# mitschabaude/msm-zprize

Hardware: AMD Instinct MI355X
Metric: Mpoint-adds/s (ms per MSM in ms_per_step) (higher is better)
Workload: dtype u32 limbs (28-bit lazy Montgomery, i64 accumulate)

## Files before the change

msm_zprize_amd/_native.py:

```python
import ctypes as C
import os

HERE = os.path.dirname(os.path.abspath(__file__))
LIB_PATH = os.environ.get("MSMZ_LIB") or os.path.join(HERE, "libmsmz.so")

MSMZ_N_STAGES = 8
STAGE_NAMES = ["digits", "scan", "scatter", "plan", "accumulate", "reduce", "final", "total"]


class MsmzOpts(C.Structure):
    _fields_ = [("c", C.c_int32), ("glv", C.c_int32), ("safe", C.c_int32), ("buckets", C.c_int32),
                ("timing", C.c_int32), ("reserved", C.c_int32 * 3)]


class MsmzLog(C.Structure):
    _fields_ = [("stage_ms", C.c_float * MSMZ_N_STAGES), ("c", C.c_int32), ("K", C.c_int32), ("rounds", C.c_int32),
                ("glv", C.c_int32), ("n_entries", C.c_uint64), ("n_pairs", C.c_uint64), ("max_bucket", C.c_uint32),
                ("scatter_launches", C.c_uint32), ("scatter_kernel_ms", C.c_float), ("batch_add_ms", C.c_float * 32)]


MSMZ_SRC_DEVICE, MSMZ_SRC_MONTGOMERY, MSMZ_SRC_DEFAULT_STREAM = 1, 2, 4


class MsmzSrc(C.Structure):
# ... 8 lines not shown
class MsmzCheckResult(C.Structure):
    _fields_ = [("off_curve", C.c_uint64), ("off_subgroup", C.c_uint64), ("first_bad", C.c_uint64)]


class MsmzMul(C.Structure):
    _fields_ = [("points_handle", C.c_uint64), ("first_p", C.c_uint64), ("scalars_handle", C.c_uint64),
                ("first_s", C.c_uint64), ("scalar", C.c_char_p), ("addend_handle", C.c_uint64), ("first_q", C.c_uint64)]


class MsmzTestReduceArgs(C.Structure):
    _fields_ = [("mode", C.c_int32), ("c", C.c_int32), ("nsets", C.c_uint32), ("n_in", C.c_uint32),
                ("nc", C.c_uint32), ("tail_n", C.c_uint32), ("quad16_max", C.c_uint32), ("pairsum_x4_max", C.c_uint32),
                ("points_xy", C.c_char_p), ("points_inf", C.c_char_p), ("n_points", C.c_uint64),
                ("slots_xy", C.c_char_p), ("slots_inf", C.c_char_p), ("n_slots", C.c_uint64),
                ("scale", C.c_char_p), ("loc", C.c_void_p), ("cscan", C.c_void_p),
                ("out_xy", C.c_void_p), ("lines_xy", C.c_void_p)]


class MsmzTestPlanArgs(C.Structure):
    _fields_ = [("nb", C.c_uint32), ("chunk", C.c_uint32), ("nb_main", C.c_uint32), ("chunk_top", C.c_uint32),
                ("tail_skip", C.c_int32), ("reserved", C.c_uint32),
                ("off", C.c_void_p), ("refs", C.c_void_p),
                ("desc_cap", C.c_uint64), ("bfin_cap", C.c_uint64), ("chunk_pairs_cap", C.c_uint64),
                ("meta", C.c_void_p), ("desc", C.c_void_p), ("bfin", C.c_void_p), ("chunk_pairs", C.c_void_p)]


class MsmzTestSortArgs(C.Structure):
    _fields_ = [("scalars_le32", C.c_void_p), ("n", C.c_uint64), ("pts_n", C.c_uint64),
                ("nprob", C.c_uint32), ("factor", C.c_uint32), ("copy_stride", C.c_uint32),
                ("c", C.c_int32), ("glv", C.c_int32), ("force_fallback", C.c_int32), ("scalar_bits", C.c_int32),
                ("allow_fold", C.c_int32),
# ... 48 lines not shown
    "msmz_test_field_limbs": (C.c_int, [C.c_void_p, C.c_int, C.c_void_p, C.c_void_p, C.c_uint64, C.c_void_p,
                                        C.c_char_p]),
    "msmz_test_glv": (C.c_int, [C.c_void_p, C.c_char_p, C.c_uint64, C.c_char_p, C.c_char_p, C.c_char_p]),
    "msmz_test_digits": (C.c_int, [C.c_void_p, C.c_char_p, C.c_uint64, C.c_int, C.c_int, C.c_int, C.c_void_p]),
    "msmz_test_sort": (C.c_int, [C.c_void_p, C.c_char_p, C.c_uint64, C.c_int, C.c_int, C.c_int, C.c_void_p, C.c_void_p,
                                 C.c_uint64, C.c_void_p, C.c_uint64]),
    "msmz_test_sort_ex": (C.c_int, [C.c_void_p, C.POINTER(MsmzTestSortArgs)]),
    "msmz_test_point_raw": (C.c_int, [C.c_void_p, C.c_int, C.c_char_p, C.c_char_p, C.c_char_p, C.c_uint64, C.c_int,
                                      C.c_char_p]),
    "msmz_test_point": (C.c_int, [C.c_void_p, C.c_int, C.c_char_p, C.c_char_p, C.c_char_p, C.c_char_p, C.c_uint64,
                                  C.c_char_p]),
    "msmz_test_batch_add": (C.c_int, [C.c_void_p, C.c_int, C.c_int, C.c_char_p, C.c_char_p, C.c_uint64, C.c_char_p,
                                      C.c_char_p, C.c_uint64, C.c_void_p, C.c_uint64, C.c_uint64, C.c_char_p,
                                      C.POINTER(C.c_uint32)]),
    "msmz_test_reduce": (C.c_int, [C.c_void_p, C.POINTER(MsmzTestReduceArgs)]),
    "msmz_test_plan": (C.c_int, [C.c_void_p, C.POINTER(MsmzTestPlanArgs)]),
}

_lib = None


class MsmzError(RuntimeError):
    def __init__(self, status, where):
        self.status = status
        msg = lib().msmz_strerror(status).decode() if _lib is not None else "?"
        super().__init__(f"{where}: msmz status {status} ({msg})")


def lib():
    global _lib
# ... 17 lines not shown
```

msm_zprize_amd/csrc/engine.h:

```cpp
#pragma once
#include <hip/hip_runtime.h>

#include <chrono>
#include <cstdio>
#include <cstdlib>
#include <cstring>
#include <map>
#include <type_traits>
#include <vector>

#include "../../include/msmz.h"
#include "kernels.h"
#include "gen_kernels.h"
#include "import_kernels.h"
#include "check_kernels.h"
#include "mul_kernels.h"
#include "host64.h"
#include "multi.h"
#include "plan.h"

namespace msmz {

#define MSMZ_HIP(x)                                                                        \
  do {                                                                                     \
// ... 118 lines not shown
    load(p, a, ai);
    load(q, b, bi);
    xyzz_add(r, p, q);
    uint32_t w[2 * NW];
    bool inf = xyzz_to_affine_canon<F>(w, r);
    memcpy(out, w, sizeof(w));
    *oi = inf ? 1 : 0;
  }
  return MSMZ_OK;
}

struct ReduceKnobs {
  uint32_t tail_n;
  uint32_t quad16_max;
  uint32_t pairsum_x4_max;
};

template <class Cfg>
class TestHooks;

template <class Cfg>
class Engine : public IEngine {
  friend class TestHooks<Cfg>;
  using F = typename Cfg::F;
  using Fr = typename Cfg::Fr;
  static constexpr int NW = F::NW;
  static constexpr int RW = 2 * NW;
  static constexpr int XW = 4 * NW;
  static constexpr int FE_BYTES = NW * 4;
  static constexpr bool TE = Cfg::TE;
  static constexpr int PW_WORDS = TE ? 4 * NW : PointFmt<F>::STRIDE;

 public:
  Engine(int curve_id, int device) : curve_id_(curve_id), device_(device) {}

  int init() {
    MSMZ_HIP(hipSetDevice(device_));
    MSMZ_HIP(hipStreamCreateWithFlags(&stream_, hipStreamNonBlocking));
    for (hipEvent_t* e : ev_.all()) MSMZ_HIP(hipEventCreate(e));
    MSMZ_HIP(hipEventCreateWithFlags(&import_ev_, hipEventDisableTiming));
    MSMZ_HIP(hipHostMalloc(&h_meta_, sizeof(MsmMeta)));
    int st;
    if ((st = ensure_host_results((size_t)2 * kMaxWindows * XW))) return st;
    if ((st = raise_lds_limit((const void*)k_fine, "k_fine", kFineLds))) return st;
    if ((st = raise_sort_limits<false, 0>()) || (st = raise_sort_limits<false, 16>()) || (st = raise_sort_limits<false, 17>())) return st;
    if constexpr (Fr::HAS_GLV) {
      if ((st = raise_sort_limits<true, 0>()) || (st = raise_sort_limits<true, 16>())) return st;
    }
    return meta_.ensure(sizeof(MsmMeta) + kTraceBytes * 65536);
  }
 private:
  template <bool GLV, int C>
  int raise_sort_limits() {
    int st;
    if ((st = raise_lds_limit((const void*)k_coarse<Fr, GLV, C>, GLV ? "k_coarse<glv>" : "k_coarse", kCoarseLdsMax))) return st;
    return raise_lds_limit((const void*)k_hist<Fr, GLV, C>, GLV ? "k_hist<glv>" : "k_hist", kHistLdsMax);
  }
  static constexpr size_t kFineLds = ((size_t)(1 << FINE_MAX_BITS) + FINE_STAGE) * 4;
  static constexpr size_t kCoarseLdsMax = (size_t)2 * SORT_MAX_BINS * 4;
  static constexpr size_t kHistLdsMax = (size_t)SORT_MAX_BINS * 4;
#ifdef MSMZ_TRACE
  static constexpr size_t kTraceBytes = 128;
#else
// ... 861 lines not shown
  }

  struct HostTe {
    using Pt = TeExt<F>;
    void set_inf(Pt& p) const { te_set_zero(p); }
    void dbl(Pt& r, const Pt& p) const { te_add(r, p, p); }
    void add_pt(Pt& r, const Pt& a, const Pt& b) const { te_add(r, a, b); }
    void load_pt(Pt& p, const uint32_t* w) const {
      fe_unpack<F>(p.X, w);
      fe_unpack<F>(p.Y, w + NW);
      fe_unpack<F>(p.Z, w + 2 * NW);
      fe_unpack<F>(p.T, w + 3 * NW);
    }
  };

  int finish_msm(const Plan& pl, Run& run, bool two_d, uint8_t* out, int* out_inf, msmz_log* log) {
    mark(run, run.ev.red_end);
    const size_t per_problem = (size_t)(two_d ? 2 : 1) * pl.Keff;
    const std::vector<WindowTerm> terms =
        window_terms(pl.c, pl.K, pl.Keff, (int)pl.F, two_d ? planner_.split_2d(pl).b : -1, pl.fold_shift != 0);
    int st = fetch_window_sums(pl, per_problem);
    if (st) return st;
    const auto t_host = std::chrono::steady_clock::now();
    if (h_meta_->error & 1u) return MSMZ_ERR_DEGENERATE;
    for (uint32_t p = 0; p < pl.nprob; p++) {
      const uint32_t* rp = h_res_ + p * per_problem * XW;
      uint32_t w[RW];
      if constexpr (TE) {
        te_to_affine_canon<F>(w, host_horner(HostTe{}, terms, rp, XW));
        out_inf[p] = 0;
      } else {
        Xyzz<F> fin;
        host64_.to_xyzz(fin, host_horner(host64_, terms, rp, XW));
        out_inf[p] = xyzz_to_affine_canon<F>(w, fin) ? 1 : 0;
      }
      memcpy(out + (size_t)p * RW * 4, w, sizeof(w));
    }
    const float host_ms = std::chrono::duration<float, std::milli>(std::chrono::steady_clock::now() - t_host).count();
    fill_log(log, pl, run, host_ms);
    return MSMZ_OK;
  }

  template <class P>
  int reduce_2d(const Plan& pl, const Split2d& sp, const ReduceKnobs& rk, const uint32_t* d_points, bool basic = false,
                bool summed = false) {
    const R2Geom g = r2_geom(pl, sp);
    int rows = 0;
    if (int st = line_sums_2d<P>(g, rk, d_points, basic, summed, &rows)) return st;
    return weighted_sums_2d<P>(g, rk, rows);
  }
  static R2Geom r2_geom(const Plan& pl, const Split2d& sp) {
    R2Geom g;
    g.L = pl.L;
    g.H = sp.H;
    g.D = sp.D;
    g.NC = sp.NC;
    g.chr = sp.D / sp.NC;
    g.chc = sp.H / sp.NC;
    g.nprob = 2u * pl.nprob * (uint32_t)pl.Keff;
    return g;
  }
  template <class P>
  int line_sums_2d(const R2Geom& g, const ReduceKnobs& rk, const uint32_t* d_points, bool basic, bool summed, int* rows) {
    const uint32_t lines = g.nprob * g.H;
// ... 3 lines not shown
    if ((st = red_[2].ensure((size_t)total * XW * 4))) return st;
    if (basic && summed) {
      hipLaunchKernelGGL((k_reduce2d_partial_acc<P>), dim3((total + 127) / 128), dim3(128), 0, stream_,
                         red_[0].as<uint32_t>(), bsum_.as<uint32_t>(), (const uint32_t*)nullptr, g, total);
    } else if (basic) {
      hipLaunchKernelGGL((k_reduce2d_partial_acc<P>), dim3((total + 127) / 128), dim3(128), 0, stream_,
                         red_[0].as<uint32_t>(), slots_.as<uint32_t>(), rscan_.as<uint32_t>(), g, total);
    } else {
      if constexpr (!TE)
        hipLaunchKernelGGL((k_reduce2d_partial<F>), dim3((total + 127) / 128), dim3(128), 0, stream_,
                           red_[0].as<uint32_t>(), slots_.as<uint32_t>(), d_points, bfin_.as<uint4>(), g, total);
    }
    int src = 0;
    for (uint32_t n = total / 2; n >= lines && g.NC > 1; n /= 2) {
      const int dst = src ^ 2;
      if (n <= rk.pairsum_x4_max) {
        hipLaunchKernelGGL((k_pairsum_x4<P>), dim3((n * 4 + 63) / 64), dim3(64), 0, stream_, red_[dst].as<uint32_t>(),
                           red_[src].as<uint32_t>(), n);
      } else {
        hipLaunchKernelGGL((k_pairsum<P>), dim3((n + 127) / 128), dim3(128), 0, stream_, red_[dst].as<uint32_t>(),
                           red_[src].as<uint32_t>(), n);
      }
      src = dst;
      if (n == lines) break;
    }
    *rows = src;
    return MSMZ_OK;
  }
  template <class P>
  int weighted_sums_2d(const R2Geom& g, const ReduceKnobs& rk, int crow) {
    const uint32_t lines = g.nprob * g.H;
    const int ccol = crow + 1;
    int st;
    if ((st = red_[ccol].ensure((size_t)lines * XW * 4))) return st;
    hipLaunchKernelGGL((k_fill_neutral<P>), dim3((lines + 255) / 256), dim3(256), 0, stream_, red_[ccol].as<uint32_t>(), lines);
    int cur = crow >> 1;
    if ((st = reduce_levels<P>(rk, cur, g.H, g.nprob))) return st;
    MSMZ_HIP(hipGetLastError());
    return MSMZ_OK;
  }
  static void fill_log(msmz_log* log, const Plan& pl, const Run& run, float host_ms) {
    if (!log) return;
    log->c = pl.c;
    log->K = pl.K;
    log->rounds = (int)run.rounds;
    log->glv = pl.glv ? 1 : 0;
    log->n_entries = run.n_entries;
    log->n_pairs = run.n_pairs;
// ... 80 lines not shown
      if (pairs == 0) continue;
      launch_batch_add(pairs, opt.safe != 0, d_points, desc_.as<uint2>() + run.round_base[r], run.round_base[r], d_meta);
#ifdef MSMZ_TRACE
      {
        char nm[32];
        snprintf(nm, sizeof nm, "k_batch_add round %d", r);
        const int B = batch_b(pairs);
        const uint32_t wgs = (pairs + MSMZ_BATCH_T * B - 1) / (MSMZ_BATCH_T * B);
        if ((st = trace_dump(nm, d_meta + 1, wgs < 65536 ? wgs : 65536, false))) return st;
      }
#endif
      mark(run, run.ev.round_end[r]);
    }
    mark(run, run.ev.acc_end);

    if (want_2d) {
      if ((st = reduce_2d<WeierPolicy<F>>(pl, planner_.split_2d(pl), reduce_knobs_, d_points))) return st;
    } else {
      uint32_t S1 = planner_.first_group_size(pl);
      if (S1 > 8) S1 = 8;
      while (S1 > 1 && S1 * 2 > pl.L) S1 >>= 1;
      const uint32_t groups = (pl.L + S1 - 1) / S1;
      if ((st = red_[0].ensure((size_t)pl.Keff * groups * XW * 4))) return st;
      if ((st = red_[1].ensure((size_t)pl.Keff * groups * XW * 4))) return st;
      if ((st = reduce_first_affine(pl, d_points, S1, groups, run.n_pairs, d_meta))) return st;
      int cur = 0;
      if ((st = reduce_levels<WeierPolicy<F>>(reduce_knobs_, cur, groups, (uint32_t)pl.Keff))) return st;
    }
    return finish_msm(pl, run, want_2d, out, out_inf, log);
  }

  int msm_basic(const Handle& pts, const uint32_t* d_points, const uint32_t* d_scalars, uint64_t n64, const msmz_opts& opt,
                uint8_t* out, int* out_inf, msmz_log* log) {
    using P = typename std::conditional<TE, TePolicy<F>, WeierPolicy<F>>::type;
    if (opt.glv) return MSMZ_ERR_UNSUPPORTED;
    Plan pl;
    int st = planner_.make_plan(pl, n64, false, opt, (uint32_t)pts.n, false);
    if (st) return st;
    Run run = new_run(opt);
    if ((st = sort_phase(pl, planner_.sort_layout(pl), d_scalars, run, 0)) || (st = fetch_meta(run))) return st;
    if (h_meta_->error & 4u) return MSMZ_ERR_RANGE;
    run.n_pairs = run.n_entries;
    if ((st = partials_.ensure((size_t)32 * pl.nblocks * 4))) return st;
    constexpr int AW = P::ACC_WORDS;
// ... 11 lines not shown
    hipLaunchKernelGGL(k_scan_apply, dim3(nblocks, 1), dim3(SCAN_T), 0, stream_, rscan_.as<uint32_t>(),
                       partials_.as<uint32_t>(), off_.as<uint32_t>(), nb, scan_mode, nblocks, (size_t)0, (uint32_t*)nullptr);
    MSMZ_HIP(hipMemcpyAsync(h_meta_, d_meta, sizeof(MsmMeta), hipMemcpyDeviceToHost, stream_));
    MSMZ_HIP(hipStreamSynchronize(stream_));
    const uint32_t n_chunks = h_meta_->round_pairs[0];
    mark(run, run.ev.plan_end);
    if ((st = slots_.ensure((size_t)(n_chunks + 1) * AW * 4))) return st;
    if (n_chunks > 0) {
      hipLaunchKernelGGL((k_bucket_accumulate<P>), dim3((n_chunks + 127) / 128), dim3(128), 0, stream_,
                         slots_.as<uint32_t>(), d_points, refs_.as<uint32_t>(), off_.as<uint32_t>(),
                         rscan_.as<uint32_t>(), nb, n_chunks, chunk_shift);
    }
    mark(run, run.ev.acc_end);
    const bool summed = (uint64_t)n_chunks * 2 > (uint64_t)nb * 3 && !no_bucket_sums_;
    if (summed && (st = bucket_sums<P>(nb))) return st;
    if ((st = reduce_2d<P>(pl, planner_.split_2d(pl), reduce_knobs_, d_points, true, summed))) return st;
    return finish_msm(pl, run, true, out, out_inf, log);
  }
  template <class P>
  int bucket_sums(uint32_t nb) {
    if (int st = bsum_.ensure((size_t)nb * P::ACC_WORDS * 4)) return st;
    hipLaunchKernelGGL((k_bucket_sums<P>), dim3((nb + 127) / 128), dim3(128), 0, stream_, bsum_.as<uint32_t>(),
                       slots_.as<uint32_t>(), rscan_.as<uint32_t>(), nb);
    return MSMZ_OK;
  }

  int reduce_first_affine(const Plan& pl, const uint32_t* d_points, uint32_t S, uint32_t groups, uint64_t tree_pairs,
                          MsmMeta* d_meta) {
    F2Geom g;
    memset(&g, 0, sizeof(g));
    g.L = pl.L;
    g.S = S;
// ... 136 lines not shown
  int curve_id_, device_;
  hipStream_t stream_ = nullptr;
  StageEvents ev_{};
  hipEvent_t import_ev_ = nullptr;
  std::vector<uint8_t> import_pack_;
  std::map<uint64_t, Handle> handles_;
  uint64_t next_handle_ = 1;
#ifdef MSMZ_DEV
  static int env_int(const char* name, int dflt) { const char* v = getenv(name); return v ? atoi(v) : dflt; }
#else
  static int env_int(const char*, int dflt) { return dflt; }
#endif
  uint32_t batch_min_wgs_ = (uint32_t)env_int("MSMZ_BATCH_WGS", 512);
  int chunk_shift_override_ = env_int("MSMZ_CHUNK_SHIFT", 0);
  const ReduceKnobs reduce_knobs_{(uint32_t)env_int("MSMZ_TAIL_N", REDUCE_TAIL_N), (uint32_t)env_int("MSMZ_QUAD16", 8192),
                                  (uint32_t)env_int("MSMZ_PAIRSUM_X4", 16384)};
  Host64<F> host64_;
  bool no_bucket_sums_ = env_int("MSMZ_NO_BUCKET_SUMS", 0) != 0;
  int tail_skip_2d_ = env_int("MSMZ_TAIL_SKIP_2D", 1) > 2 ? 2 : env_int("MSMZ_TAIL_SKIP_2D", 1);
  int batch_b_override_ = env_int("MSMZ_BATCH_B", 0);
  int retries_ = 0;
  Planner<Fr> planner_{{env_int("MSMZ_NO_SPREAD", 0) != 0, env_int("MSMZ_NO_FOLD", 0) != 0,
                        env_int("MSMZ_NO_WINDOW_MODEL", 0) != 0, env_int("MSMZ_ATOMIC_SORT", 0) != 0,
                        env_int("MSMZ_NO_FBT", 0) != 0, env_int("MSMZ_NO_PLAN_TOP", 0) != 0,
                        env_int("MSMZ_NO_SORT_SPECIAL", 0) != 0, env_int("MSMZ_FB", 0), (uint32_t)env_int("MSMZ_S1", 0),
                        (uint32_t)env_int("MSMZ_R2_NC", 0)}};
  DevBuf bsum_, f2desc_, tilecnt_, tileoff_, final_, desc_, bfin_, packed_, bins_, digits_, counts_, off_, cursor_, refs_, rscan_, partials_, slots_, red_[4], meta_, stage_, gen_table_;
  MsmMeta* h_meta_ = nullptr;
  DevBuf check_;
  CheckResult* h_check_ = nullptr;
  size_t h_check_bytes_ = 0;
  int ensure_host_check(size_t verdict_bytes) {
    const size_t need = sizeof(CheckResult) + verdict_bytes;
    if (need <= h_check_bytes_) return MSMZ_OK;
    if (h_check_) (void)hipHostFree(h_check_);
    h_check_ = nullptr;
    h_check_bytes_ = 0;
    MSMZ_HIP(hipHostMalloc(&h_check_, need));
    h_check_bytes_ = need;
    return MSMZ_OK;
  }
// ... 16 lines not shown
```

msm_zprize_amd/csrc/host64.h:

```cpp
#pragma once
#include <cstdint>
#include <cstring>
#include <vector>

#include "fp.h"

namespace msmz {

template <class F>
struct Fe64 {
  static constexpr int NL = F::NW / 2;
  uint64_t l[NL];
};

template <class F>
struct Host64 {
  static constexpr int NL = F::NW / 2;
  static constexpr int RBITS = F::N * F::W;
  static constexpr int TAIL = RBITS - 64 * NL;
  static_assert(TAIL > 0 && TAIL < 64, "radix must exceed the 64-bit limb length by less than one limb");
  using E = Fe64<F>;
  typedef unsigned __int128 u128;

  uint64_t p[NL];
// ... 218 lines not shown
  }
  std::vector<WindowTerm> t;
  for (int k = K - 1; k >= 0; k--) {
    const int top = k == K - 1 ? Keff - 1 : k;
    if (split_b < 0) {
      for (int kw = top; kw >= k; kw--) t.push_back({c * k, kw});
      continue;
    }
    if (!fold || k < K - 1)
      for (int kw = k; kw <= top; kw++) t.push_back({c * k + split_b, 2 * kw});
    for (int kw = k; kw <= top; kw++) t.push_back({c * k, 2 * kw + 1});
  }
  return t;
}

template <class G>
typename G::Pt host_horner(const G& g, const std::vector<WindowTerm>& terms, const uint32_t* res, int rec_words) {
  typename G::Pt acc, w, t;
  g.set_inf(acc);
  int prev = terms.empty() ? 0 : terms[0].weight;
  for (const WindowTerm& term : terms) {
    for (; prev > term.weight; prev--) {
      g.dbl(t, acc);
      acc = t;
    }
    g.load_pt(w, res + (size_t)term.index * rec_words);
    g.add_pt(t, acc, w);
    acc = t;
  }
  for (; prev > 0; prev--) {
// ... 8 lines not shown
```

msm_zprize_amd/csrc/instantiate.h:

```cpp
#pragma once
#include "check_kernels.h"
#include "gen_kernels.h"
#include "import_kernels.h"
#include "kernels.h"
#include "mul_kernels.h"
#include "test_kernels.h"

#if !defined(MSMZ_CURVE) || MSMZ_CURVE == 0
#define MSMZ_W0(X) X(Bls377Fp, Bls377Fr)
#else
#define MSMZ_W0(X)
#endif
#if !defined(MSMZ_CURVE) || MSMZ_CURVE == 1
#define MSMZ_W1(X) X(PallasFp, PallasFr)
#else
#define MSMZ_W1(X)
#endif
#if !defined(MSMZ_CURVE) || MSMZ_CURVE == 2
#define MSMZ_W2(X) X(Bls381Fp, Bls381Fr)
#else
#define MSMZ_W2(X)
#endif
#if !defined(MSMZ_CURVE) || MSMZ_CURVE == 3
#define MSMZ_T3(X) X(Ed377Fp, Ed377Fr)
// ... 19 lines not shown
  PFX template __global__ void k_batch_add<F, MSMZ_BATCH_T, false, MSMZ_BATCH_OCC, MSMZ_BATCH_BMAX>(             \
      uint32_t*, const uint32_t*, const uint2*, uint32_t, uint32_t, int, MsmMeta*);

#define MSMZ_INST_POLICY(P, PFX)                                                                                 \
  PFX template __global__ void k_reduce_quad<P>(uint32_t*, uint32_t*, const uint32_t*, const uint32_t*, uint32_t, \
                                                uint32_t, uint32_t);                                             \
  PFX template __global__ void k_reduce_quad16<P>(uint32_t*, uint32_t*, const uint32_t*, const uint32_t*,        \
                                                  uint32_t, uint32_t, uint32_t);                                 \
  PFX template __global__ void k_reduce_tail<P>(uint32_t*, uint32_t*, uint32_t*, uint32_t*, uint32_t*, uint32_t, \
                                                uint32_t);                                                       \
  PFX template __global__ void k_pairsum<P>(uint32_t*, const uint32_t*, uint32_t);                               \
  PFX template __global__ void k_fill_neutral<P>(uint32_t*, uint32_t);                                           \
  PFX template __global__ void k_bucket_sums<P>(uint32_t*, const uint32_t*, const uint32_t*, uint32_t);          \
  PFX template __global__ void k_reduce2d_partial_acc<P>(uint32_t*, const uint32_t*, const uint32_t*, R2Geom, uint32_t); \
  PFX template __global__ void k_pairsum_x4<P>(uint32_t*, const uint32_t*, uint32_t);                            \
  PFX template __global__ void k_bucket_accumulate<P>(uint32_t*, const uint32_t*, const uint32_t*,               \
                                                      const uint32_t*, const uint32_t*, uint32_t, uint32_t, int);

#define MSMZ_INST_REDUCE(F, Fr, PFX)                                                                              \
  PFX template __global__ void k_reduce2d_partial<F>(uint32_t*, const uint32_t*, const uint32_t*, const uint4*,   \
                                                     R2Geom, uint32_t);                                          \
  PFX template __global__ void k_reduce_affine_finish<F>(uint32_t*, uint32_t*, const uint32_t*, const uint32_t*,  \
                                                         const uint2*, const uint4*, F2Geom);                     \
  MSMZ_INST_POLICY(WeierPolicy<F>, PFX)

#define MSMZ_INST_REDUCE_TE(F, Fr, PFX) MSMZ_INST_POLICY(TePolicy<F>, PFX)

#define MSMZ_INST_TEST(F, Fr, P, TE, PFX)                                                                         \
  PFX template __global__ void k_test_field<F>(uint32_t*, const uint32_t*, const uint32_t*, uint32_t, int, uint32_t*); \
  PFX template __global__ void k_test_field_limbs<F>(int32_t*, uint32_t*, const int32_t*, const int32_t*, uint32_t,  \
// ... 62 lines not shown
```

msm_zprize_amd/csrc/kernels.h:

```cpp
#pragma once
#include <hip/hip_runtime.h>
#include "constants_gen.h"
#include "plan.h"
#include "curve.h"
#include "scalar.h"

namespace msmz {

constexpr uint32_t REF_NEG = 0x80000000u;
constexpr uint32_t REF_IDX = 0x7fffffffu;

struct MsmMeta {
  uint32_t max_bucket;
  uint32_t n_entries;
  uint32_t error;
  uint32_t rounds;
  uint32_t round_pairs[32];
  uint32_t round_base[32];
};

typedef uint32_t u32x4 __attribute__((ext_vector_type(4)));

#ifndef MSMZ_POINT_PAD
#define MSMZ_POINT_PAD 1
// ... 995 lines not shown
                                                         const uint32_t* c_in, uint32_t n_in, uint32_t groups,
                                                         uint32_t total) {
  constexpr int XW = P::ACC_WORDS;
  const uint32_t t = blockIdx.x * blockDim.x + threadIdx.x;
  const uint32_t grp = t >> 4, q = (t >> 2) & 3;
  const int s = (int)(t & 3);
  const bool live = grp < total;
  const uint32_t k = live ? grp / groups : 0, A = live ? grp - k * groups : 0;
  const int lane = threadIdx.x & 63, base_lane = (lane & ~15) + s;
  reduce_group16<P>(rows_out + (size_t)k * groups * XW, c_out + (size_t)k * groups * XW,
                    rows_in + (size_t)k * n_in * XW, c_in + (size_t)k * n_in * XW, n_in, A, live, q, s, base_lane);
}

constexpr int REDUCE_TAIL_T = 256;
constexpr uint32_t REDUCE_TAIL_N = 32;
template <class P>
__global__ void __launch_bounds__(REDUCE_TAIL_T, 1) k_reduce_tail(uint32_t* r0, uint32_t* c0, uint32_t* r1, uint32_t* c1,
                                                                  uint32_t* c_final, uint32_t n_in, uint32_t stride) {
  constexpr int XW = P::ACC_WORDS;
  const uint32_t k = blockIdx.x;
  uint32_t* rin = r0 + (size_t)k * stride * XW;
  uint32_t* cin = c0 + (size_t)k * stride * XW;
  uint32_t* rout = r1 + (size_t)k * stride * XW;
  uint32_t* cout = c1 + (size_t)k * stride * XW;
  const uint32_t q = (threadIdx.x >> 2) & 3;
  const int s = (int)(threadIdx.x & 3);
  const int lane = threadIdx.x & 63, base_lane = (lane & ~15) + s;
  uint32_t n = n_in;
  while (n > 1) {
    const uint32_t g2 = (n + 3) / 4;
    for (uint32_t A0 = 0; A0 < g2; A0 += REDUCE_TAIL_T / 16) {
      const uint32_t A = A0 + (threadIdx.x >> 4);
      reduce_group16<P>(rout, cout, rin, cin, n, A, A < g2, q, s, base_lane);
    }
    __syncthreads();
    uint32_t* t1 = rin; rin = rout; rout = t1;
    uint32_t* t2 = cin; cin = cout; cout = t2;
    n = g2;
  }
  for (uint32_t j = threadIdx.x; j < (uint32_t)XW; j += REDUCE_TAIL_T) c_final[(size_t)k * XW + j] = cin[j];
}


}

#include "reduce_affine.h"
#include "reduce2d_kernels.h"
```

msm_zprize_amd/csrc/msmz.hip:

```cpp
#include "instantiate.h"
namespace msmz {
#define X(F, Fr) MSMZ_INST_BATCH(F, Fr, MSMZ_EXTERN) MSMZ_INST_REDUCE(F, Fr, MSMZ_EXTERN) MSMZ_INST_MISC(F, Fr, MSMZ_EXTERN) MSMZ_INST_GEN(F, Fr, MSMZ_EXTERN)
MSMZ_WEIERSTRASS_FIELDS(X)
#undef X
#define X(F, Fr) MSMZ_INST_REDUCE_TE(F, Fr, MSMZ_EXTERN) MSMZ_INST_MISC_TE(F, Fr, MSMZ_EXTERN) MSMZ_INST_GEN_TE(F, Fr, MSMZ_EXTERN)
MSMZ_TE_FIELDS(X)
#undef X
}
#include "test_hooks.h"

namespace msmz {

template <class F_, class Fr_>
struct WeierCfg {
  using F = F_;
  using Fr = Fr_;
  static constexpr bool TE = false;
  static constexpr bool HAS_ENDO = true;
};

template <class F_, class Fr_>
struct TeCfg {
  using F = F_;
  using Fr = Fr_;
// ... 207 lines not shown
  return c ? c->engine->test_hooks()->test_point_raw(op, a, b, neg, n, L, out) : MSMZ_ERR_ARG;
}
int msmz_test_point(msmz_ctx* c, int op, const uint8_t* a, const uint8_t* ai, const uint8_t* b, const uint8_t* bi,
                    uint64_t n, uint8_t* out) {
  return c ? c->engine->test_hooks()->test_point(op, a, ai, b, bi, n, out) : MSMZ_ERR_ARG;
}

int msmz_test_batch_add(msmz_ctx* c, int safe, int B, const uint8_t* pxy, const uint8_t* pinf, uint64_t np,
                        const uint8_t* sxy, const uint8_t* sinf, uint64_t ns, const uint32_t* desc, uint64_t n_pairs,
                        uint64_t out_base, uint8_t* out, uint32_t* error) {
  if (!c) return MSMZ_ERR_ARG;
  return c->engine->test_hooks()->test_batch_add(safe, B, pxy, pinf, np, sxy, sinf, ns, desc, n_pairs, out_base, out, error);
}

int msmz_test_reduce(msmz_ctx* c, const msmz_test_reduce_args* a) {
  return c && a ? c->engine->test_hooks()->test_reduce(*a) : MSMZ_ERR_ARG;
}

int msmz_test_plan(msmz_ctx* c, const msmz_test_plan_args* a) {
  return c && a ? c->engine->test_hooks()->test_plan(*a) : MSMZ_ERR_ARG;
}

int msmz_point_add(int curve_id, const uint8_t* a, int ai, const uint8_t* b, int bi, uint8_t* out, int* oi) {
  if (!out || !oi || (!a && !ai) || (!b && !bi)) return MSMZ_ERR_ARG;
  switch (curve_id) {
    case MSMZ_BLS12_377_G1: return host_point_add<Bls377Fp, false>(a, ai, b, bi, out, oi);
    case MSMZ_PALLAS: return host_point_add<PallasFp, false>(a, ai, b, bi, out, oi);
    case MSMZ_BLS12_381_G1: return host_point_add<Bls381Fp, false>(a, ai, b, bi, out, oi);
    case MSMZ_ED_ON_BLS12_377: return host_point_add<Ed377Fp, true>(a, 0, b, 0, out, oi);
    default: return MSMZ_ERR_UNSUPPORTED;
  }
// ... 4 lines not shown
```

msm_zprize_amd/csrc/plan.h:

```cpp
#pragma once
#include <cstdint>
#include <cstring>

#include "../../include/msmz.h"
#include "multi.h"

namespace msmz {

constexpr int COARSE_T = 1024;
constexpr int COARSE_ITEMS = 2;
constexpr int COARSE_TILE = COARSE_T * COARSE_ITEMS;
constexpr int COARSE_MAX_BINS = 512;
constexpr int SORT_MAX_BINS = 8192;
constexpr int FINE_MAX_BITS = 11;
constexpr int FINE_T = 1024;
constexpr int FINE_PER = 37;
constexpr int FINE_STAGE = FINE_T * FINE_PER;

constexpr int PLAN_T = 512;
constexpr int PLAN_PER = 2;
constexpr int PLAN_CHUNK = PLAN_T * PLAN_PER;
constexpr int PLAN_RMAX = 26;

constexpr int SCAN_T = 256;
// ... 60 lines not shown
  uint32_t nprob = 1;
  uint32_t F = 1;
  int sbits = 0;
};

struct Geometry {
  int c, K, t_top, spread, Keff;
  uint32_t L;
  uint32_t top_range = 0;
  int fold_shift = 0, fold_rows = 0;
};

struct Split2d {
  int a, b;
  uint32_t H, D, NC;
};

struct SortLayout {
  SortGeom geom{};
  uint32_t nbins = 0, fbins = 0, fine_top = 0;
  int cspec = 0;
  bool fits = false, two_level = false;
};

struct PlanKnobs {
  bool no_spread = false, no_fold = false, no_window_model = false, force_atomic_sort = false;
  bool no_fbt = false;
  bool no_plan_top = false;
  bool no_sort_special = false;
  int fb_cap = 0;
  uint32_t s1_override = 0, r2_nc = 0;
  int glv_bits_assumed = 0;
};

template <class Fr>
struct Planner {
  PlanKnobs k;

  static int bound(int bits) { return bits <= 0 || bits >= Fr::BITS ? 0 : bits; }

  int scalar_bits(bool glv, int extra_bits, int sbits = 0) const {
    const int sb = bound(sbits);
    if (!glv) return sb ? sb : Fr::BITS;
    if (extra_bits) return Fr::GLV_PROVEN_BITS > Fr::GLV_BITS - 1 ? Fr::GLV_PROVEN_BITS : Fr::GLV_BITS - 1;
    const int a = k.glv_bits_assumed > 0 ? k.glv_bits_assumed : Fr::GLV_BITS - 1;
    return sb && sb < a ? sb : a;
  }
// ... 230 lines not shown
  }

  Split2d split_2d(const Plan& pl) const {
    Split2d s;
    s.a = (pl.c - 1 + 1) / 2;
    s.b = pl.c - 1 - s.a;
    s.H = 1u << s.a;
    s.D = 1u << s.b;
    uint32_t nc = 1;
    while (nc < 32 && nc * 2 <= s.D && (uint64_t)2 * pl.nprob * pl.Keff * s.H * nc < (1u << 18)) nc *= 2;
    if (k.r2_nc > 0) {
      nc = 1;
      while (nc < k.r2_nc && nc * 2 <= s.D) nc *= 2;
    }
    s.NC = nc;
    return s;
  }

  uint32_t batch_size(uint64_t n, const msmz_opts& opt, uint32_t pts_n, uint32_t factor, uint32_t remaining) const {
    uint32_t bs = remaining;
    for (int it = 0; it < 4 && bs > 1; it++) {
      Plan pl;
      if (make_plan(pl, n, opt.glv != 0, opt, pts_n, true, 0, true, bs, factor > 1 ? factor : 1) != MSMZ_OK) {
        bs = (bs + 1) / 2;
        continue;
      }
      const uint32_t fit = batch_split(remaining, (uint64_t)pl.K * pl.M, kMaxBatchEntries);
      if (fit >= bs) break;
      bs = fit;
    }
// ... 42 lines not shown
```

msm_zprize_amd/csrc/reduce2d_kernels.h:

```cpp
#pragma once
#include "plan.h"

namespace msmz {

template <class F>
__global__ void __launch_bounds__(128, MSMZ_REDUCE_OCC) k_reduce2d_partial(uint32_t* part, const uint32_t* slots,
                                                                           const uint32_t* points, const uint4* bfin,
                                                                           R2Geom g, uint32_t total) {
  const uint32_t t = blockIdx.x * blockDim.x + threadIdx.x;
  if (t >= total) return;
  const uint32_t per_prob = g.H * g.NC;
  const uint32_t prob = t / per_prob, u = t - prob * per_prob;
  const uint32_t kw = prob >> 1;
  const bool col = (prob & 1u) != 0;
  uint32_t line, chunk, j0 = 0, step = 0, count = 0;
  if (!col) {
    line = u / g.NC;
    chunk = u - line * g.NC;
    j0 = line * g.D + chunk;
    step = g.NC;
    count = g.chr;
  } else if (u < g.D * g.NC) {
    chunk = u / g.D;
    line = u - chunk * g.D;
// ... 133 lines not shown
  const uint32_t t = blockIdx.x * blockDim.x + threadIdx.x;
  const uint32_t i = t >> 2;
  const int s = (int)(t & 3);
  const bool live = i < n_out;
  typename P::Acc a, b, r;
  P::zero(a);
  P::zero(b);
  if (live) {
    P::load(a, in + (size_t)(2 * i) * XW);
    P::load(b, in + (size_t)(2 * i + 1) * XW);
  }
  P::add_x4(r, a, b, s, false);
  if (live && s == 0) P::store(out + (size_t)i * XW, r);
}

}
```

Baseline: 4677.

## Add split-square weighted-sum reduction kernel with LDS-resident pair trees

Adds k_weighted_sq, which reduces each 2D problem's line sums inside one workgroup. It uses LDS pair trees over two factor axes (G and H/G), so the column/weighted pass is split into two half-weight sums that the host recombines through extended window terms. The aim is to replace the multi-launch fill-neutral/column/tail reduction with a single kernel per problem and fewer point additions. The cost is large LDS use, one workgroup per problem (low parallelism), and four results per problem fetched to the host. A fused k_line_sums kernel is also added, but LINE_SUMS_MAX is 0, so it is disabled by default.

```diff
diff --git a/msm_zprize_amd/_native.py b/msm_zprize_amd/_native.py
--- a/msm_zprize_amd/_native.py
+++ b/msm_zprize_amd/_native.py
@@ -46,7 +46,7 @@
                 ("points_xy", C.c_char_p), ("points_inf", C.c_char_p), ("n_points", C.c_uint64),
                 ("slots_xy", C.c_char_p), ("slots_inf", C.c_char_p), ("n_slots", C.c_uint64),
                 ("scale", C.c_char_p), ("loc", C.c_void_p), ("cscan", C.c_void_p),
-                ("out_xy", C.c_void_p), ("lines_xy", C.c_void_p)]
+                ("out_xy", C.c_void_p), ("lines_xy", C.c_void_p), ("route", C.c_uint32)]
 
 
 class MsmzTestPlanArgs(C.Structure):
@@ -125,6 +125,7 @@
                                       C.c_char_p, C.c_uint64, C.c_void_p, C.c_uint64, C.c_uint64, C.c_char_p,
                                       C.POINTER(C.c_uint32)]),
     "msmz_test_reduce": (C.c_int, [C.c_void_p, C.POINTER(MsmzTestReduceArgs)]),
+    "msmz_test_reduce_ex": (C.c_int, [C.c_void_p, C.POINTER(MsmzTestReduceArgs), C.c_size_t]),
     "msmz_test_plan": (C.c_int, [C.c_void_p, C.POINTER(MsmzTestPlanArgs)]),
 }
 
diff --git a/msm_zprize_amd/csrc/engine.h b/msm_zprize_amd/csrc/engine.h
--- a/msm_zprize_amd/csrc/engine.h
+++ b/msm_zprize_amd/csrc/engine.h
@@ -156,6 +156,8 @@
   uint32_t tail_n;
   uint32_t quad16_max;
   uint32_t pairsum_x4_max;
+  bool weighted_sq = true;
+  uint32_t line_sums_max = LINE_SUMS_MAX;
 };
 
 template <class Cfg>
@@ -171,6 +173,7 @@
   static constexpr int XW = 4 * NW;
   static constexpr int FE_BYTES = NW * 4;
   static constexpr bool TE = Cfg::TE;
+  using RedPolicy = typename std::conditional<TE, TePolicy<F>, WeierPolicy<F>>::type;
   static constexpr int PW_WORDS = TE ? 4 * NW : PointFmt<F>::STRIDE;
 
  public:
@@ -183,12 +186,13 @@
     MSMZ_HIP(hipEventCreateWithFlags(&import_ev_, hipEventDisableTiming));
     MSMZ_HIP(hipHostMalloc(&h_meta_, sizeof(MsmMeta)));
     int st;
-    if ((st = ensure_host_results((size_t)2 * kMaxWindows * XW))) return st;
+    if ((st = ensure_host_results((size_t)4 * kMaxWindows * XW))) return st;
     if ((st = raise_lds_limit((const void*)k_fine, "k_fine", kFineLds))) return st;
     if ((st = raise_sort_limits<false, 0>()) || (st = raise_sort_limits<false, 16>()) || (st = raise_sort_limits<false, 17>())) return st;
     if constexpr (Fr::HAS_GLV) {
       if ((st = raise_sort_limits<true, 0>()) || (st = raise_sort_limits<true, 16>())) return st;
     }
+    if ((st = raise_lds_limit((const void*)k_weighted_sq<RedPolicy>, "k_weighted_sq", WSQ_LDS_BUDGET))) return st;
     return meta_.ensure(sizeof(MsmMeta) + kTraceBytes * 65536);
   }
  private:
@@ -1080,11 +1084,11 @@
     }
   };
 
-  int finish_msm(const Plan& pl, Run& run, bool two_d, uint8_t* out, int* out_inf, msmz_log* log) {
+  int finish_msm(const Plan& pl, Run& run, bool two_d, int split_g, uint8_t* out, int* out_inf, msmz_log* log) {
     mark(run, run.ev.red_end);
-    const size_t per_problem = (size_t)(two_d ? 2 : 1) * pl.Keff;
-    const std::vector<WindowTerm> terms =
-        window_terms(pl.c, pl.K, pl.Keff, (int)pl.F, two_d ? planner_.split_2d(pl).b : -1, pl.fold_shift != 0);
+    const size_t per_problem = (size_t)(two_d ? (split_g > 0 ? 4 : 2) : 1) * pl.Keff;
+    const std::vector<WindowTerm> terms = window_terms_split(pl.c, pl.K, pl.Keff, (int)pl.F, two_d ? planner_.split_2d(pl).b : -1,
+                                                             pl.fold_shift != 0, two_d ? split_g : 0);
     int st = fetch_window_sums(pl, per_problem);
     if (st) return st;
     const auto t_host = std::chrono::steady_clock::now();
@@ -1108,12 +1112,19 @@
   }
 
   template <class P>
-  int reduce_2d(const Plan& pl, const Split2d& sp, const ReduceKnobs& rk, const uint32_t* d_points, bool basic = false,
-                bool summed = false) {
+  int reduce_2d(const Plan& pl, const Split2d& sp, const ReduceKnobs& rk, const uint32_t* d_points, int* split_g,
+                bool basic = false, bool summed = false) {
     const R2Geom g = r2_geom(pl, sp);
     int rows = 0;
     if (int st = line_sums_2d<P>(g, rk, d_points, basic, summed, &rows)) return st;
-    return weighted_sums_2d<P>(g, rk, rows);
+    *split_g = wsq_split<P>(g, sp, rk);
+    return weighted_sums_2d<P>(g, rk, rows, *split_g);
+  }
+  static constexpr uint32_t WSQ_MAX_PROBLEMS = 256;
+  template <class P>
+  static int wsq_split(const R2Geom& g, const Split2d& sp, const ReduceKnobs& rk) {
+    if (!rk.weighted_sq || sp.g < 1 || g.H < 4 || g.nprob > WSQ_MAX_PROBLEMS) return 0;
+    return wsq_lds_bytes(g.H, sp.g, P::ACC_WORDS) <= WSQ_LDS_BUDGET ? sp.g : 0;
   }
   static R2Geom r2_geom(const Plan& pl, const Split2d& sp) {
     R2Geom g;
@@ -1147,6 +1158,14 @@
     int src = 0;
     for (uint32_t n = total / 2; n >= lines && g.NC > 1; n /= 2) {
       const int dst = src ^ 2;
+      int left = 1;
+      while ((n >> (left - 1)) > lines) left++;
+      if (n <= rk.line_sums_max && left <= LS_MAX_LEVELS) {
+        hipLaunchKernelGGL((k_line_sums<P>), dim3((2 * n + LS_REC - 1) / LS_REC), dim3(LS_T), 0, stream_,
+                           red_[dst].as<uint32_t>(), red_[src].as<uint32_t>(), 2 * n, left);
+        src = dst;
+        break;
+      }
       if (n <= rk.pairsum_x4_max) {
         hipLaunchKernelGGL((k_pairsum_x4<P>), dim3((n * 4 + 63) / 64), dim3(64), 0, stream_, red_[dst].as<uint32_t>(),
                            red_[src].as<uint32_t>(), n);
@@ -1161,10 +1180,17 @@
     return MSMZ_OK;
   }
   template <class P>
-  int weighted_sums_2d(const R2Geom& g, const ReduceKnobs& rk, int crow) {
+  int weighted_sums_2d(const R2Geom& g, const ReduceKnobs& rk, int crow, int split_g) {
     const uint32_t lines = g.nprob * g.H;
     const int ccol = crow + 1;
     int st;
+    if (split_g > 0) {
+      if ((st = final_.ensure((size_t)2 * g.nprob * XW * 4))) return st;
+      hipLaunchKernelGGL((k_weighted_sq<P>), dim3(g.nprob), dim3(WSQ_T), wsq_lds_bytes(g.H, split_g, P::ACC_WORDS), stream_,
+                         final_.as<uint32_t>(), red_[crow].as<uint32_t>(), g.H, split_g);
+      MSMZ_HIP(hipGetLastError());
+      return MSMZ_OK;
+    }
     if ((st = red_[ccol].ensure((size_t)lines * XW * 4))) return st;
     hipLaunchKernelGGL((k_fill_neutral<P>), dim3((lines + 255) / 256), dim3(256), 0, stream_, red_[ccol].as<uint32_t>(), lines);
     int cur = crow >> 1;
@@ -1275,8 +1301,9 @@
     }
     mark(run, run.ev.acc_end);
 
+    int split_g = 0;
     if (want_2d) {
-      if ((st = reduce_2d<WeierPolicy<F>>(pl, planner_.split_2d(pl), reduce_knobs_, d_points))) return st;
+      if ((st = reduce_2d<WeierPolicy<F>>(pl, planner_.split_2d(pl), reduce_knobs_, d_points, &split_g))) return st;
     } else {
       uint32_t S1 = planner_.first_group_size(pl);
       if (S1 > 8) S1 = 8;
@@ -1288,7 +1315,7 @@
       int cur = 0;
       if ((st = reduce_levels<WeierPolicy<F>>(reduce_knobs_, cur, groups, (uint32_t)pl.Keff))) return st;
     }
-    return finish_msm(pl, run, want_2d, out, out_inf, log);
+    return finish_msm(pl, run, want_2d, split_g, out, out_inf, log);
   }
 
   int msm_basic(const Handle& pts, const uint32_t* d_points, const uint32_t* d_scalars, uint64_t n64, const msmz_opts& opt,
@@ -1330,8 +1357,9 @@
     mark(run, run.ev.acc_end);
     const bool summed = (uint64_t)n_chunks * 2 > (uint64_t)nb * 3 && !no_bucket_sums_;
     if (summed && (st = bucket_sums<P>(nb))) return st;
-    if ((st = reduce_2d<P>(pl, planner_.split_2d(pl), reduce_knobs_, d_points, true, summed))) return st;
-    return finish_msm(pl, run, true, out, out_inf, log);
+    int split_g = 0;
+    if ((st = reduce_2d<P>(pl, planner_.split_2d(pl), reduce_knobs_, d_points, &split_g, true, summed))) return st;
+    return finish_msm(pl, run, true, split_g, out, out_inf, log);
   }
   template <class P>
   int bucket_sums(uint32_t nb) {
@@ -1498,7 +1526,8 @@
   uint32_t batch_min_wgs_ = (uint32_t)env_int("MSMZ_BATCH_WGS", 512);
   int chunk_shift_override_ = env_int("MSMZ_CHUNK_SHIFT", 0);
   const ReduceKnobs reduce_knobs_{(uint32_t)env_int("MSMZ_TAIL_N", REDUCE_TAIL_N), (uint32_t)env_int("MSMZ_QUAD16", 8192),
-                                  (uint32_t)env_int("MSMZ_PAIRSUM_X4", 16384)};
+                                  (uint32_t)env_int("MSMZ_PAIRSUM_X4", 16384), env_int("MSMZ_WSQ", 1) != 0,
+                                  (uint32_t)env_int("MSMZ_LINE_SUMS", (int)LINE_SUMS_MAX)};
   Host64<F> host64_;
   bool no_bucket_sums_ = env_int("MSMZ_NO_BUCKET_SUMS", 0) != 0;
   int tail_skip_2d_ = env_int("MSMZ_TAIL_SKIP_2D", 1) > 2 ? 2 : env_int("MSMZ_TAIL_SKIP_2D", 1);
@@ -1508,7 +1537,7 @@
                         env_int("MSMZ_NO_WINDOW_MODEL", 0) != 0, env_int("MSMZ_ATOMIC_SORT", 0) != 0,
                         env_int("MSMZ_NO_FBT", 0) != 0, env_int("MSMZ_NO_PLAN_TOP", 0) != 0,
                         env_int("MSMZ_NO_SORT_SPECIAL", 0) != 0, env_int("MSMZ_FB", 0), (uint32_t)env_int("MSMZ_S1", 0),
-                        (uint32_t)env_int("MSMZ_R2_NC", 0)}};
+                        (uint32_t)env_int("MSMZ_R2_NC", 0), 0, env_int("MSMZ_NO_SPLIT_SQ", 0) != 0}};
   DevBuf bsum_, f2desc_, tilecnt_, tileoff_, final_, desc_, bfin_, packed_, bins_, digits_, counts_, off_, cursor_, refs_, rscan_, partials_, slots_, red_[4], meta_, stage_, gen_table_;
   MsmMeta* h_meta_ = nullptr;
   DevBuf check_;
diff --git a/msm_zprize_amd/csrc/host64.h b/msm_zprize_amd/csrc/host64.h
--- a/msm_zprize_amd/csrc/host64.h
+++ b/msm_zprize_amd/csrc/host64.h
@@ -1,6 +1,7 @@
 #pragma once
 #include <cstdint>
 #include <cstring>
+#include <algorithm>
 #include <vector>
 
 #include "fp.h"
@@ -256,6 +257,18 @@
   return t;
 }
 
+static inline std::vector<WindowTerm> window_terms_split(int c, int K, int Keff, int F, int split_b, bool fold, int split_g) {
+  const std::vector<WindowTerm> base = window_terms(c, K, Keff, F, split_b, fold);
+  if (split_g <= 0 || split_b < 0) return base;
+  std::vector<WindowTerm> t;
+  for (const WindowTerm& w : base) {
+    t.push_back({w.weight + split_g, 2 * w.index});
+    t.push_back({w.weight, 2 * w.index + 1});
+  }
+  std::stable_sort(t.begin(), t.end(), [](const WindowTerm& x, const WindowTerm& y) { return x.weight > y.weight; });
+  return t;
+}
+
 template <class G>
 typename G::Pt host_horner(const G& g, const std::vector<WindowTerm>& terms, const uint32_t* res, int rec_words) {
   typename G::Pt acc, w, t;
diff --git a/msm_zprize_amd/csrc/instantiate.h b/msm_zprize_amd/csrc/instantiate.h
--- a/msm_zprize_amd/csrc/instantiate.h
+++ b/msm_zprize_amd/csrc/instantiate.h
@@ -57,6 +57,8 @@
   PFX template __global__ void k_bucket_sums<P>(uint32_t*, const uint32_t*, const uint32_t*, uint32_t);          \
   PFX template __global__ void k_reduce2d_partial_acc<P>(uint32_t*, const uint32_t*, const uint32_t*, R2Geom, uint32_t); \
   PFX template __global__ void k_pairsum_x4<P>(uint32_t*, const uint32_t*, uint32_t);                            \
+  PFX template __global__ void k_line_sums<P>(uint32_t*, const uint32_t*, uint32_t, int);                        \
+  PFX template __global__ void k_weighted_sq<P>(uint32_t*, const uint32_t*, uint32_t, int);                      \
   PFX template __global__ void k_bucket_accumulate<P>(uint32_t*, const uint32_t*, const uint32_t*,               \
                                                       const uint32_t*, const uint32_t*, uint32_t, uint32_t, int);
 
diff --git a/msm_zprize_amd/csrc/kernels.h b/msm_zprize_amd/csrc/kernels.h
--- a/msm_zprize_amd/csrc/kernels.h
+++ b/msm_zprize_amd/csrc/kernels.h
@@ -1033,31 +1033,38 @@
 
 constexpr int REDUCE_TAIL_T = 256;
 constexpr uint32_t REDUCE_TAIL_N = 32;
+template <class P, int T>
+__device__ __forceinline__ const uint32_t* reduce_tail_levels(uint32_t* rin, uint32_t* cin, uint32_t* rout, uint32_t* cout,
+                                                              uint32_t n, uint32_t nfam, uint32_t stride) {
+  constexpr int XW = P::ACC_WORDS;
+  const uint32_t q = (threadIdx.x >> 2) & 3;
+  const int s = (int)(threadIdx.x & 3);
+  const int lane = threadIdx.x & 63, base_lane = (lane & ~15) + s;
+  while (n > 1) {
+    const uint32_t g2 = (n + 3) / 4, total = nfam * g2;
+    for (uint32_t A0 = 0; A0 < total; A0 += T / 16) {
+      const uint32_t Af = A0 + (threadIdx.x >> 4);
+      const bool live = Af < total;
+      const uint32_t fam = live ? Af / g2 : 0, A = Af - fam * g2;
+      const size_t o = (size_t)fam * stride * XW;
+      reduce_group16<P>(rout + o, cout + o, rin + o, cin + o, n, A, live, q, s, base_lane);
+    }
+    __syncthreads();
+    uint32_t* t1 = rin; rin = rout; rout = t1;
+    uint32_t* t2 = cin; cin = cout; cout = t2;
+    n = g2;
+  }
+  return cin;
+}
+
 template <class P>
 __global__ void __launch_bounds__(REDUCE_TAIL_T, 1) k_reduce_tail(uint32_t* r0, uint32_t* c0, uint32_t* r1, uint32_t* c1,
                                                                   uint32_t* c_final, uint32_t n_in, uint32_t stride) {
   constexpr int XW = P::ACC_WORDS;
   const uint32_t k = blockIdx.x;
-  uint32_t* rin = r0 + (size_t)k * stride * XW;
-  uint32_t* cin = c0 + (size_t)k * stride * XW;
-  uint32_t* rout = r1 + (size_t)k * stride * XW;
-  uint32_t* cout = c1 + (size_t)k * stride * XW;
-  const uint32_t q = (threadIdx.x >> 2) & 3;
-  const int s = (int)(threadIdx.x & 3);
-  const int lane = threadIdx.x & 63, base_lane = (lane & ~15) + s;
-  uint32_t n = n_in;
-  while (n > 1) {
-    const uint32_t g2 = (n + 3) / 4;
-    for (uint32_t A0 = 0; A0 < g2; A0 += REDUCE_TAIL_T / 16) {
-      const uint32_t A = A0 + (threadIdx.x >> 4);
-      reduce_group16<P>(rout, cout, rin, cin, n, A, A < g2, q, s, base_lane);
-    }
-    __syncthreads();
-    uint32_t* t1 = rin; rin = rout; rout = t1;
-    uint32_t* t2 = cin; cin = cout; cout = t2;
-    n = g2;
-  }
-  for (uint32_t j = threadIdx.x; j < (uint32_t)XW; j += REDUCE_TAIL_T) c_final[(size_t)k * XW + j] = cin[j];
+  const size_t o = (size_t)k * stride * XW;
+  const uint32_t* res = reduce_tail_levels<P, REDUCE_TAIL_T>(r0 + o, c0 + o, r1 + o, c1 + o, n_in, 1, 0);
+  for (uint32_t j = threadIdx.x; j < (uint32_t)XW; j += REDUCE_TAIL_T) c_final[(size_t)k * XW + j] = res[j];
 }
 
 
diff --git a/msm_zprize_amd/csrc/msmz.hip b/msm_zprize_amd/csrc/msmz.hip
--- a/msm_zprize_amd/csrc/msmz.hip
+++ b/msm_zprize_amd/csrc/msmz.hip
@@ -245,7 +245,13 @@
 }
 
 int msmz_test_reduce(msmz_ctx* c, const msmz_test_reduce_args* a) {
-  return c && a ? c->engine->test_hooks()->test_reduce(*a) : MSMZ_ERR_ARG;
+  return c && a ? c->engine->test_hooks()->test_reduce(*a, MSMZ_TR_ROUTE_DEFAULT) : MSMZ_ERR_ARG;
+}
+
+int msmz_test_reduce_ex(msmz_ctx* c, const msmz_test_reduce_args* a, size_t args_size) {
+  if (!c || !a || args_size < offsetof(msmz_test_reduce_args, route)) return MSMZ_ERR_ARG;
+  const uint32_t route = args_size >= offsetof(msmz_test_reduce_args, route) + sizeof(a->route) ? a->route : MSMZ_TR_ROUTE_DEFAULT;
+  return c->engine->test_hooks()->test_reduce(*a, route);
 }
 
 int msmz_test_plan(msmz_ctx* c, const msmz_test_plan_args* a) {
diff --git a/msm_zprize_amd/csrc/plan.h b/msm_zprize_amd/csrc/plan.h
--- a/msm_zprize_amd/csrc/plan.h
+++ b/msm_zprize_amd/csrc/plan.h
@@ -98,6 +98,7 @@
 struct Split2d {
   int a, b;
   uint32_t H, D, NC;
+  int g = 0;
 };
 
 struct SortLayout {
@@ -115,6 +116,7 @@
   int fb_cap = 0;
   uint32_t s1_override = 0, r2_nc = 0;
   int glv_bits_assumed = 0;
+  bool no_split_sq = false;
 };
 
 template <class Fr>
@@ -375,6 +377,7 @@
       while (nc < k.r2_nc && nc * 2 <= s.D) nc *= 2;
     }
     s.NC = nc;
+    s.g = (!k.no_split_sq && s.a >= 2) ? s.a / 2 : 0;
     return s;
   }
 
diff --git a/msm_zprize_amd/csrc/reduce2d_kernels.h b/msm_zprize_amd/csrc/reduce2d_kernels.h
--- a/msm_zprize_amd/csrc/reduce2d_kernels.h
+++ b/msm_zprize_amd/csrc/reduce2d_kernels.h
@@ -171,4 +171,118 @@
   if (live && s == 0) P::store(out + (size_t)i * XW, r);
 }
 
-}
+constexpr int LS_T = 256;
+constexpr uint32_t LS_REC = LS_T / 2;
+constexpr int LS_MAX_LEVELS = 7;
+constexpr uint32_t LINE_SUMS_MAX = 0;
+template <class P>
+__global__ void __launch_bounds__(LS_T, 1) k_line_sums(uint32_t* out, const uint32_t* in, uint32_t n_in, int levels) {
+  constexpr int XW = P::ACC_WORDS;
+  static_assert(XW % 4 == 0 && (LS_T / 4) * XW * 4 <= (64 << 10), "k_line_sums: LDS records");
+  __shared__ __attribute__((aligned(16))) uint32_t lds[(LS_T / 4) * XW];
+  const uint32_t q = threadIdx.x >> 2;
+  const int s = (int)(threadIdx.x & 3);
+  const uint32_t base = blockIdx.x * LS_REC;
+  uint32_t n = (n_in - base < LS_REC ? n_in - base : LS_REC) >> 1;
+  typename P::Acc a, b, r;
+  P::zero(a);
+  P::zero(b);
+  if (q < n) {
+    P::load(a, in + (size_t)(base + 2 * q) * XW);
+    P::load(b, in + (size_t)(base + 2 * q + 1) * XW);
+  }
+  P::add_x4(r, a, b, s, false);
+  for (int level = 1; level < levels; level++) {
+    if (q < n && s == 0) P::store(lds + (size_t)q * XW, r);
+    __syncthreads();
+    n >>= 1;
+    P::zero(a);
+    P::zero(b);
+    if (q < n) {
+      P::load(a, lds + (size_t)(2 * q) * XW);
+      P::load(b, lds + (size_t)(2 * q + 1) * XW);
+    }
+    __syncthreads();
+    P::add_x4(r, a, b, s, false);
+  }
+  if (q < n && s == 0) P::store(out + (size_t)((base >> levels) + q) * XW, r);
+}
+
+constexpr int WSQ_T = 256;
+constexpr uint32_t WSQ_LDS_BUDGET = 128u << 10;
+constexpr size_t wsq_lds_bytes(uint32_t H, int g, int acc_words) {
+  return ((size_t)H + H / 2 + 8 * (size_t)(H >> g)) * acc_words * 4;
+}
+
+template <class P>
+__device__ __forceinline__ void wsq_pair_level(uint32_t* out0, uint32_t* out1, const uint32_t* in0, const uint32_t* in1,
+                                               uint32_t n0, uint32_t n1, bool transposed, uint32_t G, uint32_t half_gp) {
+  constexpr int XW = P::ACC_WORDS;
+  const int s = (int)(threadIdx.x & 3);
+  const uint32_t total = n0 + n1;
+  for (uint32_t j0 = 0; j0 < total; j0 += WSQ_T / 4) {
+    const uint32_t j = j0 + (threadIdx.x >> 2);
+    const bool live = j < total, f1 = j >= n0;
+    const uint32_t i = f1 ? j - n0 : j;
+    uint32_t ia = 2 * i, ib = 2 * i + 1;
+    if (f1 && transposed) {
+      const uint32_t v = i / half_gp, e = i - v * half_gp;
+      ia = 2 * e * G + v;
+      ib = ia + G;
+    }
+    const uint32_t* in = f1 ? in1 : in0;
+    typename P::Acc a, b, r;
+    P::zero(a);
+    P::zero(b);
+    if (live) {
+      P::load(a, in + (size_t)ia * XW);
+      P::load(b, in + (size_t)ib * XW);
+    }
+    P::add_x4(r, a, b, s, false);
+    if (live && s == 0) P::store((f1 ? out1 : out0) + (size_t)i * XW, r);
+  }
+}
+
+template <class P>
+__global__ void __launch_bounds__(WSQ_T, 1) k_weighted_sq(uint32_t* c_final, const uint32_t* rows, uint32_t H, int g) {
+  constexpr int XW = P::ACC_WORDS;
+  extern __shared__ uint4 wsq_lds[];
+  uint32_t* lds = reinterpret_cast<uint32_t*>(wsq_lds);
+  const uint32_t G = 1u << g, Gp = H >> g;
+  const uint32_t* R = rows + (size_t)blockIdx.x * H * XW;
+  auto pp = [&](uint32_t f, uint32_t b) { return lds + (size_t)((b ? H : 0u) + (f ? (b ? H / 4 : H / 2) : 0u)) * XW; };
+  uint32_t* tail = lds + (size_t)(H + H / 2) * XW;
+  uint32_t* rin = tail;
+  uint32_t* cin = rin + (size_t)2 * Gp * XW;
+  uint32_t* rout = cin + (size_t)2 * Gp * XW;
+  uint32_t* cout = rout + (size_t)2 * Gp * XW;
+  for (uint32_t i = threadIdx.x; i < 4 * Gp; i += WSQ_T) {
+    typename P::Acc z;
+    P::zero(z);
+    P::store(rin + (size_t)i * XW, z);
+  }
+  __syncthreads();
+  uint32_t e0 = G, e1 = Gp;
+  const uint32_t* in0 = R;
+  const uint32_t* in1 = R;
+  for (int level = 0; e0 > 1 || e1 > 1; level++) {
+    const uint32_t n0 = e0 > 1 ? Gp * (e0 / 2) : 0, n1 = e1 > 1 ? G * (e1 / 2) : 0;
+    uint32_t* o0 = e0 == 2 ? rin : pp(0, level & 1);
+    uint32_t* o1 = e1 == 2 ? rin + (size_t)Gp * XW : pp(1, level & 1);
+    wsq_pair_level<P>(o0, o1, in0, in1, n0, n1, level == 0, G, Gp / 2);
+    __syncthreads();
+    if (e0 > 1) {
+      e0 /= 2;
+      in0 = o0;
+    }
+    if (e1 > 1) {
+      e1 /= 2;
+      in1 = o1;
+    }
+  }
+  const uint32_t* res = reduce_tail_levels<P, WSQ_T>(rin, cin, rout, cout, Gp, 2, Gp);
+  for (uint32_t j = threadIdx.x; j < 2u * XW; j += WSQ_T)
+    c_final[(size_t)2 * blockIdx.x * XW + j] = res[(size_t)(j / XW) * Gp * XW + j % XW];
+}
+
+}
```

Result: no change. 4702 (median of 2 runs) (+0.5%).
